# Geo3DSmart/PDANet

Measured on AMD Instinct MI355X. Metric: scenes/sec (16384-pt ONCE, PDA-SSD forward+backward), higher is better.
Workload: dtype f32; 1 GPU; once16k_b2_detector_fwd_bwd_adam; scenes_per_gpu=2, global_batch=2, parallelism=dp1, world_size_seen=1, cpu_affinity=GPU-local NUMA node of 0000:f4:00.0: 128 CPUs, full=False, graph_tail=False, graph_head=True

## Files before the change

### pdanet_amd/csrc/group_attention.hip

```cpp
#include "pda_common.h"

namespace pda {

typedef float f32x16 __attribute__((ext_vector_type(16)));

__device__ __forceinline__ int acc_row(int r, int h) { return (r & 3) + 8 * (r >> 2) + 4 * h; }

template <int HD>
struct GaPtrs {
    __device__ __forceinline__ static size_t qkv(int H, size_t row, int which, int head) {
        return ((row * 3 + which) * H + head) * (size_t)HD;
    }
    __device__ __forceinline__ static size_t o(int H, size_t row, int head) { return (row * H + head) * (size_t)HD; }
};

template <int HD>
struct Tile {
    static constexpr int LD = HD + 4;
    static constexpr int LPR = HD / 4;
    static constexpr int RPI = 64 / LPR;
    static constexpr int NI = HD / 8;

    template <class TIO, class RowOff>
    __device__ __forceinline__ static void load(float4 (&raw)[NI], const TIO* base, RowOff row_off, int lane) {
#pragma unroll
        for (int it = 0; it < NI; ++it) {
            bool valid;
            const unsigned o = row_off(it * RPI + lane / LPR, valid) + 4u * (unsigned)(lane % LPR);
            const float4 v = load4(base + o);
            raw[it] = valid ? v : make_float4(0.f, 0.f, 0.f, 0.f);
        }
    }
    __device__ __forceinline__ static void to_operand(float (&dst)[HD / 2], const float4 (&raw)[NI], float* lds, int lane) {
#pragma unroll
        for (int it = 0; it < NI; ++it)
            *reinterpret_cast<float4*>(lds + (it * RPI + lane / LPR) * LD + 4 * (lane % LPR)) = raw[it];
        const float* src = lds + (lane & 31) * LD + (lane >> 5) * (HD / 2);
#pragma unroll
        for (int q = 0; q < HD / 8; ++q) {
            const float4 v = *reinterpret_cast<const float4*>(src + 4 * q);
            dst[4 * q + 0] = v.x; dst[4 * q + 1] = v.y; dst[4 * q + 2] = v.z; dst[4 * q + 3] = v.w;
        }
    }
    __device__ __forceinline__ static void from_acc(float* lds, const f32x16& acc, int dblk, int lane) {
        float* dst = lds + (lane & 31) * LD + dblk * 32 + 4 * (lane >> 5);
#pragma unroll
        for (int q = 0; q < 4; ++q)
            *reinterpret_cast<float4*>(dst + 8 * q) = make_float4(acc[4 * q], acc[4 * q + 1], acc[4 * q + 2], acc[4 * q + 3]);
    }
    template <class TIO, class RowOff>
    __device__ __forceinline__ static void store(const float* lds, TIO* base, RowOff row_off, int lane) {
#pragma unroll
        for (int it = 0; it < NI; ++it) {
            const int r = it * RPI + lane / LPR;
            bool valid;
            const unsigned o = row_off(r, valid) + 4u * (unsigned)(lane % LPR);
            const float4 v = *reinterpret_cast<const float4*>(lds + r * LD + 4 * (lane % LPR));
            if (valid) store4(base + o, v);
        }
    }
};

template <int S, int HD, bool BWD, typename TIO, bool RAGGED>
__device__ __forceinline__ void group_attention_tile(const TIO* __restrict__ qkv, const TIO* __restrict__ dout,
                                                     TIO* __restrict__ out, float* __restrict__ lse, TIO* __restrict__ dqkv,
                                                     int H, int head, float scale, float* lds, int lane, int64_t base, int rows,
                                                     int lo, int n, int64_t gid) {
    using TL = Tile<HD>;
    const int c = lane & 31, h2 = lane >> 5;
    const bool ok = c < rows;
    const int sl = c - lo;
    const TIO* qb = qkv + GaPtrs<HD>::qkv(H, (size_t)base, 0, head);
    const TIO* dob = BWD ? dout + GaPtrs<HD>::o(H, (size_t)base, head) : nullptr;
    const unsigned OS = (unsigned)(H * HD), RS = 3u * OS;
    auto in_row = [&](int which) {
        return [&, which](int r, bool& valid) -> unsigned {
            valid = r < rows;
            return (valid ? (unsigned)r * RS : 0u) + (unsigned)which * OS;
        };
    };
    auto o_row = [&](int r, bool& valid) -> unsigned {
        valid = r < rows;
        return valid ? (unsigned)r * OS : 0u;
    };
    auto key_ok = [&](int j) -> bool { return j >= lo && j < lo + n; };
    const float lnw = (RAGGED && ok) ? __logf((float)(S - n + 1)) : 0.f;

    float kq[HD / 2], qq[HD / 2];
    {
        float4 rk[TL::NI], rq[TL::NI];
        TL::load(rk, qb, in_row(1), lane);
        TL::load(rq, qb, in_row(0), lane);
        TL::to_operand(kq, rk, lds, lane);
        TL::to_operand(qq, rq, lds, lane);
    }
    f32x16 T;
#pragma unroll
    for (int i = 0; i < 16; ++i) T[i] = 0.f;
#pragma unroll
    for (int t = 0; t < HD / 2; ++t) T = __builtin_amdgcn_mfma_f32_32x32x2f32(kq[t], qq[t], T, 0, 0, 0);

    float lse_i;
    f32x16 P;
    if (!BWD) {
        float m = -__builtin_inff();
#pragma unroll
        for (int r = 0; r < 16; ++r) {
            const int j = acc_row(r, h2);
            T[r] = key_ok(j) ? T[r] * scale : -__builtin_inff();
            m = fmaxf(m, T[r]);
        }
        m = fmaxf(m, __shfl_xor(m, 32));
        float l = 0.f;
#pragma unroll
        for (int r = 0; r < 16; ++r) {
            P[r] = __expf((T[r] - m) + ((RAGGED && acc_row(r, h2) == lo) ? lnw : 0.f));
            l += P[r];
        }
        l += __shfl_xor(l, 32);
        const float inv = 1.f / l;
#pragma unroll
        for (int r = 0; r < 16; ++r) P[r] *= inv;
        lse_i = m + __logf(l);
        if (ok && h2 == 0) lse[(gid * H + head) * S + sl] = lse_i;
    } else {
        lse_i = ok ? lse[(gid * H + head) * S + sl] : 0.f;
#pragma unroll
        for (int r = 0; r < 16; ++r) {
            const int j = acc_row(r, h2);
            P[r] = key_ok(j) ? __expf((T[r] * scale - lse_i) + ((RAGGED && j == lo) ? lnw : 0.f)) : 0.f;
        }
        float l = 0.f;
#pragma unroll
        for (int r = 0; r < 16; ++r) l += P[r];
        l += __shfl_xor(l, 32);
        const float inv = l > 0.f ? 1.f / l : 0.f;
#pragma unroll
        for (int r = 0; r < 16; ++r) P[r] *= inv;
    }

    auto key_val = [&](int which, int t, int col) -> float {
        bool valid;
        const unsigned o = in_row(which)(acc_row(t, h2), valid) + (unsigned)col;
        const float v = load1(qb + o);
        return valid ? v : 0.f;
    };

    if (!BWD) {
#pragma unroll
        for (int dblk = 0; dblk < HD / 32; ++dblk) {
            f32x16 O;
#pragma unroll
            for (int i = 0; i < 16; ++i) O[i] = 0.f;
#pragma unroll
            for (int t = 0; t < 16; ++t) {
                O = __builtin_amdgcn_mfma_f32_32x32x2f32(key_val(2, t, dblk * 32 + c), P[t], O, 0, 0, 0);
            }
            TL::from_acc(lds, O, dblk, lane);
        }
        TL::store(lds, out + GaPtrs<HD>::o(H, (size_t)base, head), o_row, lane);
    } else {
        float vv[HD / 2], dd[HD / 2];
        {
            float4 rv[TL::NI], rd[TL::NI];
            TL::load(rv, qb, in_row(2), lane);
            TL::load(rd, dob, o_row, lane);
            TL::to_operand(vv, rv, lds, lane);
            TL::to_operand(dd, rd, lds, lane);
        }
        f32x16 dP;
#pragma unroll
        for (int i = 0; i < 16; ++i) dP[i] = 0.f;
#pragma unroll
        for (int t = 0; t < HD / 2; ++t) dP = __builtin_amdgcn_mfma_f32_32x32x2f32(vv[t], dd[t], dP, 0, 0, 0);
        float delta = 0.f;
#pragma unroll
        for (int r = 0; r < 16; ++r) delta += P[r] * dP[r];
        delta += __shfl_xor(delta, 32);
        f32x16 dS;
#pragma unroll
        for (int r = 0; r < 16; ++r) dS[r] = P[r] * (dP[r] - delta) * scale;

        float* tp = lds;
        float* ts = lds + 32 * 33;
#pragma unroll
        for (int r = 0; r < 16; ++r) {
            tp[acc_row(r, h2) * 33 + c] = P[r];
            ts[acc_row(r, h2) * 33 + c] = dS[r];
        }
        float Pn[16], dSn[16];
#pragma unroll
        for (int t = 0; t < 16; ++t) {
            Pn[t] = tp[c * 33 + acc_row(t, h2)];
            dSn[t] = ts[c * 33 + acc_row(t, h2)];
        }
        auto qry_o_val = [&](int t, int col) -> float {
            bool valid;
            const unsigned o = o_row(acc_row(t, h2), valid) + (unsigned)col;
            const float v = load1(dob + o);
            return valid ? v : 0.f;
        };
        TIO* dqb = dqkv + GaPtrs<HD>::qkv(H, (size_t)base, 0, head);
#pragma unroll
        for (int dblk = 0; dblk < HD / 32; ++dblk) {
            f32x16 acc;
#pragma unroll
            for (int i = 0; i < 16; ++i) acc[i] = 0.f;
#pragma unroll
            for (int t = 0; t < 16; ++t) {
                acc = __builtin_amdgcn_mfma_f32_32x32x2f32(key_val(1, t, dblk * 32 + c), dS[t], acc, 0, 0, 0);
            }
            TL::from_acc(lds, acc, dblk, lane);
        }
        TL::store(lds, dqb, in_row(0), lane);
#pragma unroll
        for (int dblk = 0; dblk < HD / 32; ++dblk) {
            f32x16 acc;
#pragma unroll
            for (int i = 0; i < 16; ++i) acc[i] = 0.f;
#pragma unroll
            for (int t = 0; t < 16; ++t) {
                acc = __builtin_amdgcn_mfma_f32_32x32x2f32(key_val(0, t, dblk * 32 + c), dSn[t], acc, 0, 0, 0);
            }
            TL::from_acc(lds, acc, dblk, lane);
        }
        TL::store(lds, dqb, in_row(1), lane);
#pragma unroll
        for (int dblk = 0; dblk < HD / 32; ++dblk) {
            f32x16 acc;
#pragma unroll
            for (int i = 0; i < 16; ++i) acc[i] = 0.f;
#pragma unroll
            for (int t = 0; t < 16; ++t) {
                acc = __builtin_amdgcn_mfma_f32_32x32x2f32(qry_o_val(t, dblk * 32 + c), Pn[t], acc, 0, 0, 0);
            }
            TL::from_acc(lds, acc, dblk, lane);
        }
        TL::store(lds, dqb, in_row(2), lane);
    }
}

constexpr int GA_BLOCK_ROWS = 128;
constexpr int64_t GA_MIN_WAVES = 8192;

template <int S, int HD, bool BWD, typename TIO, bool RAGGED>
__global__ __launch_bounds__(256, 2) void group_attention_kernel(const TIO* __restrict__ qkv, const TIO* __restrict__ dout,
                                                               TIO* __restrict__ out, float* __restrict__ lse,
                                                               TIO* __restrict__ dqkv, int64_t nb, int H, float scale,
                                                               const int32_t* __restrict__ cnt, const int32_t* __restrict__ off,
                                                               int kb) {
    const int KB = RAGGED ? kb : 32 / S;
    using TL = Tile<HD>;
    constexpr int TRN = 2 * 32 * 33;
    constexpr int LDSW = (BWD && TRN > 32 * TL::LD) ? TRN : 32 * TL::LD;
    __shared__ __attribute__((aligned(16))) float lds_all[4][LDSW];
    const int w = wave_id(), lane = lane_id();
    float* lds = lds_all[w];
    const int c = lane & 31;
    const int64_t task = (int64_t)blockIdx.x * 4 + w;
    const int head = (int)(task % H);
    const int64_t b0 = (task / H) * KB;
    if (b0 >= nb) return;
    if (!RAGGED) {
        const int rows = (int)min((int64_t)KB, nb - b0) * S;
        group_attention_tile<S, HD, BWD, TIO, false>(qkv, dout, out, lse, dqkv, H, head, scale, lds, lane, b0 * S, rows,
                                                     c < rows ? (c / S) * S : c, c < rows ? S : 1, b0 + c / S);
    } else {
        const int64_t bend = min(nb, b0 + (int64_t)KB);
        int64_t g = b0;
#pragma nounroll
        while (g < bend) {
            int lv = lane;
            asm volatile("" : "+v"(lv));
            const int c = lv & 31;
            const int64_t base = off[g];
            int rows = 0, lo = c, n = 1;
            int64_t gid = g;
            do {
                const int cn = min(max(cnt[g], 0), S);
                if (rows + cn > 32 || off[g] != base + rows) break;
                if (c >= rows && c < rows + cn) { lo = rows; n = cn; gid = g; }
                rows += cn;
                ++g;
            } while (g < bend);
            if (rows > 0)
                group_attention_tile<S, HD, BWD, TIO, true>(qkv, dout, out, lse, dqkv, H, head, scale, lds, lv, base, rows, lo,
                                                            n, gid);
        }
    }
}

template <bool BWD, typename TIO, bool RAGGED = false>
static int launch_group_attention(const TIO* qkv, const TIO* dout, TIO* out, float* lse, TIO* dqkv,
                                  int64_t nb, int s, int h, int hd, hipStream_t stream, const char* what,
                                  const int32_t* cnt = nullptr, const int32_t* off = nullptr, int64_t tokens = 0) {
    PDA_REQUIRE(nb >= 0 && h >= 1 && s >= 1 && s <= 32 && tokens >= 0, "%s: bad size", what);
    if (nb == 0) return PDA_OK;
    PDA_REQUIRE(qkv && lse && (BWD ? (dout && dqkv) : (out != nullptr)), "%s: null pointer", what);
    PDA_REQUIRE(!RAGGED || (cnt && off), "%s: null pointer", what);
    int G = 32 / s;
    if (RAGGED) {
        const int64_t mean = std::max<int64_t>(1, std::min<int64_t>(s, divup64(tokens, nb)));
        const int64_t cap = std::max<int64_t>(1, nb * h / GA_MIN_WAVES);
        G = (int)std::max<int64_t>(32 / mean, std::min<int64_t>(GA_BLOCK_ROWS / mean, cap));
        G = std::max(1, std::min(G, 64));
    }
    const float scale = 1.0f / sqrtf((float)hd);
    void (*kern)(const TIO*, const TIO*, TIO*, float*, TIO*, int64_t, int, float, const int32_t*, const int32_t*, int) = nullptr;
#define PDA_GA_CASE(SS, DD) if (s == SS && hd == DD) kern = group_attention_kernel<SS, DD, BWD, TIO, RAGGED>
    PDA_GA_CASE(32, 64); PDA_GA_CASE(16, 64); PDA_GA_CASE(8, 64);
    PDA_GA_CASE(32, 128); PDA_GA_CASE(16, 128); PDA_GA_CASE(8, 128);
    PDA_GA_CASE(32, 32); PDA_GA_CASE(16, 32); PDA_GA_CASE(8, 32);
#undef PDA_GA_CASE
    if (!kern) {
        set_error("%s: no kernel built for seq=%d head_dim=%d", what, s, hd);
        return PDA_ERR_UNSUPPORTED;
    }
    const int64_t tasks = divup64(nb, G) * h;
    const int64_t blocks = divup64(tasks, 4);
    PDA_REQUIRE(blocks < INT32_MAX, "%s: too many groups", what);
    hipLaunchKernelGGL(kern, dim3((unsigned)blocks), dim3(256), 0, stream, qkv, dout, out, lse, dqkv, nb, h, scale, cnt, off, G);
    return check_launch(what);
}

}

PDA_API int pda_group_attention_fwd(const float* qkv, float* out, float* lse, int64_t num_groups, int seq,
                                    int heads, int head_dim, pda_stream_t stream) {
    return pda::launch_group_attention<false, float>(qkv, nullptr, out, lse, nullptr, num_groups, seq, heads, head_dim,
                                              (hipStream_t)stream, "pda_group_attention_fwd");
}

PDA_API int pda_group_attention_bwd(const float* qkv, const float* grad_out, const float* lse, float* grad_qkv,
                                    int64_t num_groups, int seq, int heads, int head_dim, pda_stream_t stream) {
    return pda::launch_group_attention<true, float>(qkv, grad_out, nullptr, const_cast<float*>(lse), grad_qkv, num_groups,
                                             seq, heads, head_dim, (hipStream_t)stream, "pda_group_attention_bwd");
}

PDA_API int pda_group_attention_fwd_bf16(const uint16_t* qkv, uint16_t* out, float* lse, int64_t num_groups, int seq,
                                         int heads, int head_dim, pda_stream_t stream) {
    return pda::launch_group_attention<false, pda::bf16_t>(qkv, nullptr, out, lse, nullptr, num_groups, seq, heads, head_dim,
                                                           (hipStream_t)stream, "pda_group_attention_fwd_bf16");
}

PDA_API int pda_group_attention_bwd_bf16(const uint16_t* qkv, const uint16_t* grad_out, const float* lse, uint16_t* grad_qkv,
                                         int64_t num_groups, int seq, int heads, int head_dim, pda_stream_t stream) {
    return pda::launch_group_attention<true, pda::bf16_t>(qkv, grad_out, nullptr, const_cast<float*>(lse), grad_qkv, num_groups,
                                                          seq, heads, head_dim, (hipStream_t)stream, "pda_group_attention_bwd_bf16");
}

PDA_API int pda_group_attention_ragged_fwd(const float* qkv, const int32_t* cnt, const int32_t* off, float* out, float* lse,
                                           int64_t tokens, int64_t num_groups, int seq, int heads, int head_dim,
                                           pda_stream_t stream) {
    return pda::launch_group_attention<false, float, true>(qkv, nullptr, out, lse, nullptr, num_groups, seq, heads, head_dim,
                                                           (hipStream_t)stream, "pda_group_attention_ragged_fwd", cnt, off, tokens);
}

PDA_API int pda_group_attention_ragged_bwd(const float* qkv, const float* grad_out, const float* lse, const int32_t* cnt,
                                           const int32_t* off, float* grad_qkv, int64_t tokens, int64_t num_groups, int seq,
                                           int heads, int head_dim, pda_stream_t stream) {
    return pda::launch_group_attention<true, float, true>(qkv, grad_out, nullptr, const_cast<float*>(lse), grad_qkv, num_groups, seq,
                                                          heads, head_dim, (hipStream_t)stream, "pda_group_attention_ragged_bwd", cnt, off,
                                                          tokens);
}
```

Baseline: 119.1 scenes/s.

## Stage group-attention tiles through LDS, prefetch loads early, parallelise ragged packing

The second-stage matmuls now read V/K/Q/dout from a staged LDS image filled by coalesced float4 loads, replacing scattered per-element global loads. Loads for the next operand are issued before the current MFMA chain, with sched barriers, so memory latency overlaps compute. The backward pass shares a single transpose buffer, which halves LDS use and allows 3 blocks per CU when HD is 64. The serial ragged-group packing loop is replaced by a wave-wide prefix scan, a ballot and a binary search. The extra register pressure from prefetching and from masking instead of invalid-row address clamping could reduce occupancy or introduce correctness risk.

```diff
diff --git a/pdanet_amd/csrc/group_attention.hip b/pdanet_amd/csrc/group_attention.hip
--- a/pdanet_amd/csrc/group_attention.hip
+++ b/pdanet_amd/csrc/group_attention.hip
@@ -27,20 +27,31 @@
         for (int it = 0; it < NI; ++it) {
             bool valid;
             const unsigned o = row_off(it * RPI + lane / LPR, valid) + 4u * (unsigned)(lane % LPR);
-            const float4 v = load4(base + o);
-            raw[it] = valid ? v : make_float4(0.f, 0.f, 0.f, 0.f);
-        }
-    }
-    __device__ __forceinline__ static void to_operand(float (&dst)[HD / 2], const float4 (&raw)[NI], float* lds, int lane) {
-#pragma unroll
-        for (int it = 0; it < NI; ++it)
-            *reinterpret_cast<float4*>(lds + (it * RPI + lane / LPR) * LD + 4 * (lane % LPR)) = raw[it];
+            raw[it] = load4(base + o);
+        }
+    }
+    __device__ __forceinline__ static void to_image(float* lds, const float4 (&raw)[NI], int rows, int lane) {
+#pragma unroll
+        for (int it = 0; it < NI; ++it) {
+            const int r = it * RPI + lane / LPR;
+            const unsigned m = r < rows ? ~0u : 0u;
+            const float4 v = raw[it];
+            *reinterpret_cast<float4*>(lds + r * LD + 4 * (lane % LPR)) =
+                make_float4(__uint_as_float(__float_as_uint(v.x) & m), __uint_as_float(__float_as_uint(v.y) & m),
+                            __uint_as_float(__float_as_uint(v.z) & m), __uint_as_float(__float_as_uint(v.w) & m));
+        }
+    }
+    __device__ __forceinline__ static void to_operand(float (&dst)[HD / 2], const float4 (&raw)[NI], int rows, float* lds, int lane) {
+        to_image(lds, raw, rows, lane);
         const float* src = lds + (lane & 31) * LD + (lane >> 5) * (HD / 2);
 #pragma unroll
         for (int q = 0; q < HD / 8; ++q) {
             const float4 v = *reinterpret_cast<const float4*>(src + 4 * q);
             dst[4 * q + 0] = v.x; dst[4 * q + 1] = v.y; dst[4 * q + 2] = v.z; dst[4 * q + 3] = v.w;
         }
+    }
+    __device__ __forceinline__ static float acc_order(const float* lds, int t, int dblk, int lane) {
+        return lds[acc_row(t, lane >> 5) * LD + dblk * 32 + (lane & 31)];
     }
     __device__ __forceinline__ static void from_acc(float* lds, const f32x16& acc, int dblk, int lane) {
         float* dst = lds + (lane & 31) * LD + dblk * 32 + 4 * (lane >> 5);
@@ -86,13 +97,25 @@
     auto key_ok = [&](int j) -> bool { return j >= lo && j < lo + n; };
     const float lnw = (RAGGED && ok) ? __logf((float)(S - n + 1)) : 0.f;
 
+    constexpr bool EARLY = BWD && HD < 64;
+    auto fresh = [&]() -> int {
+        int l = lane;
+        asm volatile("" : "+v"(l));
+        return l;
+    };
+    float lse_i = 0.f;
+    if (BWD) lse_i = ok ? lse[(gid * H + head) * S + sl] : 0.f;
     float kq[HD / 2], qq[HD / 2];
+    float4 rv[TL::NI], rd[TL::NI];
     {
         float4 rk[TL::NI], rq[TL::NI];
-        TL::load(rk, qb, in_row(1), lane);
-        TL::load(rq, qb, in_row(0), lane);
-        TL::to_operand(kq, rk, lds, lane);
-        TL::to_operand(qq, rq, lds, lane);
+        TL::load(rk, qb, in_row(1), fresh());
+        TL::load(rq, qb, in_row(0), fresh());
+        TL::to_operand(kq, rk, rows, lds, lane);
+        TL::load(rv, qb, in_row(2), fresh());
+        if (EARLY) TL::load(rd, dob, o_row, fresh());
+        __builtin_amdgcn_sched_barrier(0);
+        TL::to_operand(qq, rq, rows, lds, lane);
     }
     f32x16 T;
 #pragma unroll
@@ -100,7 +123,8 @@
 #pragma unroll
     for (int t = 0; t < HD / 2; ++t) T = __builtin_amdgcn_mfma_f32_32x32x2f32(kq[t], qq[t], T, 0, 0, 0);
 
-    float lse_i;
+    if (BWD && !EARLY) TL::load(rd, dob, o_row, fresh());
+
     f32x16 P;
     if (!BWD) {
         float m = -__builtin_inff();
@@ -124,7 +148,6 @@
         lse_i = m + __logf(l);
         if (ok && h2 == 0) lse[(gid * H + head) * S + sl] = lse_i;
     } else {
-        lse_i = ok ? lse[(gid * H + head) * S + sl] : 0.f;
 #pragma unroll
         for (int r = 0; r < 16; ++r) {
             const int j = acc_row(r, h2);
@@ -139,40 +162,37 @@
         for (int r = 0; r < 16; ++r) P[r] *= inv;
     }
 
-    auto key_val = [&](int which, int t, int col) -> float {
-        bool valid;
-        const unsigned o = in_row(which)(acc_row(t, h2), valid) + (unsigned)col;
-        const float v = load1(qb + o);
-        return valid ? v : 0.f;
+    auto second_stage = [&](const auto& b, TIO* dst, auto dst_row) {
+        f32x16 acc[HD / 32];
+#pragma unroll
+        for (int dblk = 0; dblk < HD / 32; ++dblk) {
+#pragma unroll
+            for (int i = 0; i < 16; ++i) acc[dblk][i] = 0.f;
+#pragma unroll
+            for (int t = 0; t < 16; ++t)
+                acc[dblk] = __builtin_amdgcn_mfma_f32_32x32x2f32(TL::acc_order(lds, t, dblk, lane), b[t], acc[dblk], 0, 0, 0);
+        }
+#pragma unroll
+        for (int dblk = 0; dblk < HD / 32; ++dblk) TL::from_acc(lds, acc[dblk], dblk, lane);
+        TL::store(lds, dst, dst_row, fresh());
     };
 
     if (!BWD) {
-#pragma unroll
-        for (int dblk = 0; dblk < HD / 32; ++dblk) {
-            f32x16 O;
-#pragma unroll
-            for (int i = 0; i < 16; ++i) O[i] = 0.f;
-#pragma unroll
-            for (int t = 0; t < 16; ++t) {
-                O = __builtin_amdgcn_mfma_f32_32x32x2f32(key_val(2, t, dblk * 32 + c), P[t], O, 0, 0, 0);
-            }
-            TL::from_acc(lds, O, dblk, lane);
-        }
-        TL::store(lds, out + GaPtrs<HD>::o(H, (size_t)base, head), o_row, lane);
+        TL::to_image(lds, rv, rows, lane);
+        second_stage(P, out + GaPtrs<HD>::o(H, (size_t)base, head), o_row);
     } else {
         float vv[HD / 2], dd[HD / 2];
-        {
-            float4 rv[TL::NI], rd[TL::NI];
-            TL::load(rv, qb, in_row(2), lane);
-            TL::load(rd, dob, o_row, lane);
-            TL::to_operand(vv, rv, lds, lane);
-            TL::to_operand(dd, rd, lds, lane);
-        }
+        TL::to_operand(vv, rv, rows, lds, lane);
+        TL::to_operand(dd, rd, rows, lds, lane);
+        float4 rn[TL::NI];
+        if (EARLY) TL::load(rn, qb, in_row(1), fresh());
+        __builtin_amdgcn_sched_barrier(0);
         f32x16 dP;
 #pragma unroll
         for (int i = 0; i < 16; ++i) dP[i] = 0.f;
 #pragma unroll
         for (int t = 0; t < HD / 2; ++t) dP = __builtin_amdgcn_mfma_f32_32x32x2f32(vv[t], dd[t], dP, 0, 0, 0);
+        if (!EARLY) TL::load(rn, qb, in_row(1), fresh());
         float delta = 0.f;
 #pragma unroll
         for (int r = 0; r < 16; ++r) delta += P[r] * dP[r];
@@ -181,62 +201,26 @@
 #pragma unroll
         for (int r = 0; r < 16; ++r) dS[r] = P[r] * (dP[r] - delta) * scale;
 
-        float* tp = lds;
-        float* ts = lds + 32 * 33;
-#pragma unroll
-        for (int r = 0; r < 16; ++r) {
-            tp[acc_row(r, h2) * 33 + c] = P[r];
-            ts[acc_row(r, h2) * 33 + c] = dS[r];
-        }
+        auto transposed = [&](const f32x16& a, float (&an)[16]) {
+#pragma unroll
+            for (int r = 0; r < 16; ++r) lds[acc_row(r, h2) * 33 + c] = a[r];
+#pragma unroll
+            for (int t = 0; t < 16; ++t) an[t] = lds[c * 33 + acc_row(t, h2)];
+        };
         float Pn[16], dSn[16];
-#pragma unroll
-        for (int t = 0; t < 16; ++t) {
-            Pn[t] = tp[c * 33 + acc_row(t, h2)];
-            dSn[t] = ts[c * 33 + acc_row(t, h2)];
-        }
-        auto qry_o_val = [&](int t, int col) -> float {
-            bool valid;
-            const unsigned o = o_row(acc_row(t, h2), valid) + (unsigned)col;
-            const float v = load1(dob + o);
-            return valid ? v : 0.f;
-        };
+        transposed(P, Pn);
         TIO* dqb = dqkv + GaPtrs<HD>::qkv(H, (size_t)base, 0, head);
-#pragma unroll
-        for (int dblk = 0; dblk < HD / 32; ++dblk) {
-            f32x16 acc;
-#pragma unroll
-            for (int i = 0; i < 16; ++i) acc[i] = 0.f;
-#pragma unroll
-            for (int t = 0; t < 16; ++t) {
-                acc = __builtin_amdgcn_mfma_f32_32x32x2f32(key_val(1, t, dblk * 32 + c), dS[t], acc, 0, 0, 0);
-            }
-            TL::from_acc(lds, acc, dblk, lane);
-        }
-        TL::store(lds, dqb, in_row(0), lane);
-#pragma unroll
-        for (int dblk = 0; dblk < HD / 32; ++dblk) {
-            f32x16 acc;
-#pragma unroll
-            for (int i = 0; i < 16; ++i) acc[i] = 0.f;
-#pragma unroll
-            for (int t = 0; t < 16; ++t) {
-                acc = __builtin_amdgcn_mfma_f32_32x32x2f32(key_val(0, t, dblk * 32 + c), dSn[t], acc, 0, 0, 0);
-            }
-            TL::from_acc(lds, acc, dblk, lane);
-        }
-        TL::store(lds, dqb, in_row(1), lane);
-#pragma unroll
-        for (int dblk = 0; dblk < HD / 32; ++dblk) {
-            f32x16 acc;
-#pragma unroll
-            for (int i = 0; i < 16; ++i) acc[i] = 0.f;
-#pragma unroll
-            for (int t = 0; t < 16; ++t) {
-                acc = __builtin_amdgcn_mfma_f32_32x32x2f32(qry_o_val(t, dblk * 32 + c), Pn[t], acc, 0, 0, 0);
-            }
-            TL::from_acc(lds, acc, dblk, lane);
-        }
-        TL::store(lds, dqb, in_row(2), lane);
+        TL::to_image(lds, rn, rows, lane);
+        TL::load(rn, qb, in_row(0), fresh());
+        __builtin_amdgcn_sched_barrier(0);
+        second_stage(dS, dqb, in_row(0));
+        transposed(dS, dSn);
+        TL::to_image(lds, rn, rows, lane);
+        TL::load(rn, dob, o_row, fresh());
+        __builtin_amdgcn_sched_barrier(0);
+        second_stage(dSn, dqb, in_row(1));
+        TL::to_image(lds, rn, rows, lane);
+        second_stage(Pn, dqb, in_row(2));
     }
 }
 
@@ -244,48 +228,64 @@
 constexpr int64_t GA_MIN_WAVES = 8192;
 
 template <int S, int HD, bool BWD, typename TIO, bool RAGGED>
-__global__ __launch_bounds__(256, 2) void group_attention_kernel(const TIO* __restrict__ qkv, const TIO* __restrict__ dout,
+__global__ __launch_bounds__(256, (BWD && HD == 64) ? 3 : 2) void group_attention_kernel(const TIO* __restrict__ qkv, const TIO* __restrict__ dout,
                                                                TIO* __restrict__ out, float* __restrict__ lse,
                                                                TIO* __restrict__ dqkv, int64_t nb, int H, float scale,
                                                                const int32_t* __restrict__ cnt, const int32_t* __restrict__ off,
                                                                int kb) {
     const int KB = RAGGED ? kb : 32 / S;
     using TL = Tile<HD>;
-    constexpr int TRN = 2 * 32 * 33;
+    constexpr int TRN = 32 * 33;
     constexpr int LDSW = (BWD && TRN > 32 * TL::LD) ? TRN : 32 * TL::LD;
     __shared__ __attribute__((aligned(16))) float lds_all[4][LDSW];
     const int w = wave_id(), lane = lane_id();
     float* lds = lds_all[w];
     const int c = lane & 31;
     const int64_t task = (int64_t)blockIdx.x * 4 + w;
-    const int head = (int)(task % H);
-    const int64_t b0 = (task / H) * KB;
+    const int64_t gblk = task / H;
+    const int head = __builtin_amdgcn_readfirstlane((int)(task - gblk * H));
+    const int64_t b0 = (int64_t)(((uint64_t)(uint32_t)__builtin_amdgcn_readfirstlane((int)(gblk >> 32)) << 32) |
+                                 (uint32_t)__builtin_amdgcn_readfirstlane((int)gblk)) * KB;
     if (b0 >= nb) return;
     if (!RAGGED) {
         const int rows = (int)min((int64_t)KB, nb - b0) * S;
         group_attention_tile<S, HD, BWD, TIO, false>(qkv, dout, out, lse, dqkv, H, head, scale, lds, lane, b0 * S, rows,
                                                      c < rows ? (c / S) * S : c, c < rows ? S : 1, b0 + c / S);
     } else {
-        const int64_t bend = min(nb, b0 + (int64_t)KB);
-        int64_t g = b0;
+        const int ng = (int)(min(nb, b0 + (int64_t)KB) - b0);
+        const int cn = lane < ng ? min(max(cnt[b0 + lane], 0), S) : 0;
+        const int of = lane < ng ? off[b0 + lane] : 0;
+        int x = cn;
+#pragma unroll
+        for (int d = 1; d < 64; d <<= 1) {
+            const int v = __shfl_up(x, d);
+            if (lane >= d) x += v;
+        }
+        x -= cn;
+        int s = 0;
 #pragma nounroll
-        while (g < bend) {
+        while (s < ng) {
             int lv = lane;
             asm volatile("" : "+v"(lv));
             const int c = lv & 31;
-            const int64_t base = off[g];
-            int rows = 0, lo = c, n = 1;
-            int64_t gid = g;
-            do {
-                const int cn = min(max(cnt[g], 0), S);
-                if (rows + cn > 32 || off[g] != base + rows) break;
-                if (c >= rows && c < rows + cn) { lo = rows; n = cn; gid = g; }
-                rows += cn;
-                ++g;
-            } while (g < bend);
+            const int base = __builtin_amdgcn_readlane(of, s), xs = __builtin_amdgcn_readlane(x, s);
+            const int before = x - xs;
+            const bool fails = lv > s && lv < ng && (before + cn > 32 || of != base + before);
+            const uint64_t fm = __ballot(fails);
+            const int e = fm ? __ffsll((unsigned long long)fm) - 1 : ng;
+            const int rows = __builtin_amdgcn_readlane(x + cn, e - 1) - xs;
+            int ga = s, gb = e;
+#pragma unroll
+            for (int it = 0; it < 6; ++it) {
+                const int mid = (ga + gb) >> 1;
+                if (__shfl(x, mid) - xs <= c) ga = mid; else gb = mid;
+            }
+            const int glo = __shfl(x, ga) - xs, gn = __shfl(cn, ga);
+            const bool in = c < rows;
             if (rows > 0)
-                group_attention_tile<S, HD, BWD, TIO, true>(qkv, dout, out, lse, dqkv, H, head, scale, lds, lv, base, rows, lo,
-                                                            n, gid);
+                group_attention_tile<S, HD, BWD, TIO, true>(qkv, dout, out, lse, dqkv, H, head, scale, lds, lv, (int64_t)base, rows,
+                                                            in ? glo : c, in ? gn : 1, b0 + (in ? ga : s));
+            s = e;
         }
     }
 }
```

New measurement: 114.9 scenes/s. 3.5% lower.
